# yisol/IDM-VTON

Measured on NVIDIA H100. Metric: try-on images/sec @768x1024, 30 steps, CFG 2.0, higher is better.
Workload: dtype fp16

## Files before the change

idm-vton_b200/csrc/gemm.cu:

```cuda
#include "gemm_common.cuh"
#include "host.h"
#include "wgmma.cuh"

namespace vton {

enum : int { KIND_F16 = 0, KIND_F16IN_F32OUT = 1, KIND_TF32 = 2 };

template <int BN, int STAGES, bool SC>
struct SmemLayout {
  static constexpr int B_BYTES = BN * 128;
  static constexpr int STAGE_BYTES = A_BYTES + B_BYTES;
  static constexpr int LDS = BN + 4;
  static constexpr int STG_BYTES = 128 * LDS * 4;
  static constexpr int RING = STAGES * STAGE_BYTES;
  static constexpr int STG_TOTAL = (SC ? 2 : 1) * STG_BYTES;
  static constexpr int BAR_OFFSET = RING > STG_TOTAL ? RING : STG_TOTAL;
  static constexpr int TOTAL = BAR_OFFSET + 256 + 1024;
};

constexpr int GEMM_THREADS = 288;

template <int BN, int STAGES, bool GEGLU, bool SC, int KIND>
__global__ void __launch_bounds__(GEMM_THREADS, 1)
gemm_conv_kernel(const __grid_constant__ CUtensorMap tmA, const __grid_constant__ CUtensorMap tmB,
                 const __grid_constant__ CUtensorMap tmS0, const __grid_constant__ CUtensorMap tmS1,
                 const __grid_constant__ CUtensorMap tmBs, const GemmParams p) {
  using L = SmemLayout<BN, STAGES, SC>;
  constexpr int KBK = KIND == KIND_TF32 ? 32 : 64;
  extern __shared__ uint8_t smem_raw[];
  const uint32_t smem_base = (smem_u32(smem_raw) + 1023u) & ~1023u;
  float* stg = reinterpret_cast<float*>(smem_raw + (smem_base - smem_u32(smem_raw)));
  const uint32_t bar_base = smem_base + L::BAR_OFFSET;
  auto full_bar = [&](int s) { return bar_base + 8u * s; };
  auto empty_bar = [&](int s) { return bar_base + 8u * (STAGES + s); };

  const int warp = threadIdx.x >> 5;
  const int lane = threadIdx.x & 31;
  const int tile = blockIdx.x;
  const int n_tile = tile % p.n_tiles;
  const int m_tile = tile / p.n_tiles;
  const int n0 = n_tile * BN;
  const int total_slabs = p.slabs_main + (SC ? p.slabs_sc : 0);

  int b0 = 0, y0 = 0, x0 = 0;
  if (p.conv) {
    const int tx = m_tile % p.tiles_x;
    const int ty = (m_tile / p.tiles_x) % p.tiles_y;
    const int tb = m_tile / (p.tiles_x * p.tiles_y);
    x0 = tx * p.bw;
    y0 = ty * p.bh;
    b0 = tb * p.bb;
  }

  if (warp == 8 && lane == 0) {
    tma_prefetch_desc(&tmA);
    tma_prefetch_desc(&tmB);
    if (SC) {
      tma_prefetch_desc(&tmS0);
      tma_prefetch_desc(&tmS1);
      tma_prefetch_desc(&tmBs);
    }
    for (int s = 0; s < STAGES; ++s) {
      mbar_init(full_bar(s), 1);
      mbar_init(empty_bar(s), 2);
    }
    fence_barrier_init();
  }
  pdl_wait();
  __syncthreads();
  pdl_launch_dependents();

  if (warp == 8) {
    if (lane == 0) {
      for (int s = 0; s < total_slabs; ++s) {
        const int stage = s % STAGES;
        const uint32_t phase = (s / STAGES) & 1;
        mbar_wait(empty_bar(stage), phase ^ 1);
        const uint32_t a_dst = smem_base + stage * L::STAGE_BYTES;
        const uint32_t b_dst = a_dst + A_BYTES;
        mbar_expect_tx(full_bar(stage), L::STAGE_BYTES);
        if (s < p.slabs_main) {
          if (p.conv) {
            const int tap = s / p.cin_slabs;
            const int c0 = (s - tap * p.cin_slabs) * KBK;
            const int dy = tap / 3 - 1, dx = tap % 3 - 1;
            tma_load_4d(a_dst, &tmA, full_bar(stage), c0, x0 * p.stride + dx, y0 * p.stride + dy, b0);
            tma_load_2d(b_dst, &tmB, full_bar(stage), c0, tap * p.cout + n0);
          } else {
            tma_load_2d(a_dst, &tmA, full_bar(stage), s * KBK, m_tile * BM);
            tma_load_2d(b_dst, &tmB, full_bar(stage), s * KBK, n0);
          }
        } else {
          const int ss = s - p.slabs_main;
          if (ss < p.sc_split)
            tma_load_4d(a_dst, &tmS0, full_bar(stage), ss * BK, x0, y0, b0);
          else
            tma_load_4d(a_dst, &tmS1, full_bar(stage), (ss - p.sc_split) * BK, x0, y0, b0);
          tma_load_2d(b_dst, &tmBs, full_bar(stage), ss * BK, n0);
        }
      }
    }
    return;
  }

  const int wg = warp >> 2;
  float acc[BN / 2];
  float acc_sc[BN / 2];
  auto run_slabs = [&](float (&accr)[BN / 2], int s_begin, int s_end) {
    for (int s = s_begin; s < s_end; ++s) {
      const int stage = s % STAGES;
      mbar_wait(full_bar(stage), (s / STAGES) & 1);
      const uint32_t a_src = smem_base + stage * L::STAGE_BYTES + wg * (64 * 128);
      const uint32_t b_src = smem_base + stage * L::STAGE_BYTES + A_BYTES;
      wgmma_fence();
#pragma unroll
      for (int k = 0; k < 4; ++k) {
        const uint64_t da = make_gmma_desc_sw128(a_src + k * 32, 0, 1024);
        const uint64_t db = make_gmma_desc_sw128(b_src + k * 32, 0, 1024);
        const int scale_d = (s > s_begin || k > 0) ? 1 : 0;
        if constexpr (KIND == KIND_TF32) {
          WgmmaTF32SS<BN>::mma(accr, da, db, scale_d);
        } else {
          WgmmaF16SS<BN, 0>::mma(accr, da, db, scale_d);
        }
      }
      wgmma_commit();
      wgmma_wait<1>();
      if (s > 0 && (threadIdx.x & 127) == 0) mbar_arrive(empty_bar((s - 1) % STAGES));
    }
  };
  run_slabs(acc, 0, p.slabs_main);
  if constexpr (SC) run_slabs(acc_sc, p.slabs_main, total_slabs);
  wgmma_wait<0>();
  fence_regs(acc);
  if (SC) fence_regs(acc_sc);

  named_bar_sync(1, 256);
  {
    const int r0 = wg * 64 + ((warp & 3) << 4) + (lane >> 2);
    const int cq = (lane & 3) * 2;
#pragma unroll
    for (int i = 0; i < BN / 8; ++i) {
      *reinterpret_cast<float2*>(stg + r0 * L::LDS + i * 8 + cq) = make_float2(acc[4 * i], acc[4 * i + 1]);
      *reinterpret_cast<float2*>(stg + (r0 + 8) * L::LDS + i * 8 + cq) = make_float2(acc[4 * i + 2], acc[4 * i + 3]);
      if (SC) {
        float* s2 = stg + 128 * L::LDS;
        *reinterpret_cast<float2*>(s2 + r0 * L::LDS + i * 8 + cq) = make_float2(acc_sc[4 * i], acc_sc[4 * i + 1]);
        *reinterpret_cast<float2*>(s2 + (r0 + 8) * L::LDS + i * 8 + cq) = make_float2(acc_sc[4 * i + 2], acc_sc[4 * i + 3]);
      }
    }
  }
  named_bar_sync(1, 256);
  const int row = threadIdx.x & 127;
  const int half = threadIdx.x >> 7;
  long long out_row;
  int sample;
  map_row(p, m_tile, row, &out_row, &sample);
  const float* srow = stg + row * L::LDS;
  if (KIND == KIND_F16) {
    epilogue_store<BN, GEGLU>(p, srow, SC ? srow + 128 * L::LDS : nullptr, n_tile, out_row, sample, half, 2);
    return;
  }
  if (out_row < 0) return;
  const float* res_row = p.res_f32 ? p.res_f32 + out_row * p.N : nullptr;
#pragma unroll 1
  for (int c = half; c < BN / 32; c += 2) {
    const int ncol = n0 + c * 32;
    if (ncol >= p.N) continue;
#pragma unroll
    for (int g = 0; g < 8; ++g) {
      float4 v = *reinterpret_cast<const float4*>(srow + c * 32 + g * 4);
      if (p.bias_f32 != nullptr) {
        const float4 b4 = __ldg(reinterpret_cast<const float4*>(p.bias_f32 + ncol + g * 4));
        v.x += b4.x, v.y += b4.y, v.z += b4.z, v.w += b4.w;
      }
      if (res_row != nullptr) {
        const float4 r4 = __ldg(reinterpret_cast<const float4*>(res_row + ncol + g * 4));
        v.x += r4.x, v.y += r4.y, v.z += r4.z, v.w += r4.w;
      }
      *reinterpret_cast<float4*>(p.out_f32 + out_row * p.N + ncol + g * 4) = v;
    }
  }
}

template <int BN, int STAGES, bool GEGLU, bool SC, int KIND>
static int launch_variant(const CUtensorMap& tmA, const CUtensorMap& tmB, const CUtensorMap& tmS0,
                          const CUtensorMap& tmS1, const CUtensorMap& tmBs, const GemmParams& p, int grid,
                          cudaStream_t stream) {
  using L = SmemLayout<BN, STAGES, SC>;
  static_assert(L::TOTAL <= 227 * 1024, "shared memory budget");
  auto kern = gemm_conv_kernel<BN, STAGES, GEGLU, SC, KIND>;
  static bool configured = false;
  if (!configured) {
    VTON_CUDA(cudaFuncSetAttribute(kern, cudaFuncAttributeMaxDynamicSharedMemorySize, L::TOTAL));
    configured = true;
  }
  VTON_CUDA(launch_kernel(kern, dim3(grid), dim3(GEMM_THREADS), L::TOTAL, stream, tmA, tmB, tmS0, tmS1, tmBs, p));
  count_launch();
  return kOk;
}

void set_auto_v2(int) {}
void set_cluster4(int) {}

static int pick_bn(int N, int m_tiles, bool geglu, bool has_shortcut, int force_bn) {
  if (force_bn >= 2000) force_bn -= 2000;
  else if (force_bn >= 1000) force_bn -= 1000;
  auto usable = [&](int bn) {
    if (geglu && ((bn != 256 && bn != 128) || N % bn != 0)) return false;
    if (has_shortcut && bn > 128) return false;
    return true;
  };
  if (force_bn) {
    const bool known = force_bn == 64 || force_bn == 128 || force_bn == 160 || force_bn == 192 || force_bn == 256;
    return known && usable(force_bn) ? force_bn : 0;
  }
  const int sms = num_sms();
  const int cands[5] = {256, 192, 160, 128, 64};
  double best = 1e300;
  int best_bn = 0;
  for (int bn : cands) {
    if (!usable(bn)) continue;
    if (bn != 128 && N % bn != 0 && !(bn == 64 && N < 64)) continue;
    const long long tiles = static_cast<long long>(m_tiles) * cdiv(N, bn);
    const long long waves = (tiles + sms - 1) / sms;
    const double cost = static_cast<double>(waves) * (bn + 64);
    if (cost < best * 0.999) {
      best = cost;
      best_bn = bn;
    }
  }
  return best_bn ? best_bn : 128;
}

static int dispatch(int bn, bool geglu, const CUtensorMap& tmA, const CUtensorMap& tmB, const CUtensorMap& tmS0,
                    const CUtensorMap& tmS1, const CUtensorMap& tmBs, GemmParams& p, int m_tiles,
                    cudaStream_t stream) {
  p.n_tiles = cdiv(p.N, bn);
  const int grid = m_tiles * p.n_tiles;
  if (geglu) {
    if (bn == 128) return launch_variant<128, 6, true, false, KIND_F16>(tmA, tmB, tmS0, tmS1, tmBs, p, grid, stream);
    if (bn == 256) return launch_variant<256, 4, true, false, KIND_F16>(tmA, tmB, tmS0, tmS1, tmBs, p, grid, stream);
    set_last_error("GEGLU epilogue supports BN 128/256 only (got %d)", bn);
    return kErrUnsupported;
  }
  if (p.slabs_sc) {
    if (bn == 64) return launch_variant<64, 8, false, true, KIND_F16>(tmA, tmB, tmS0, tmS1, tmBs, p, grid, stream);
    if (bn == 128) return launch_variant<128, 6, false, true, KIND_F16>(tmA, tmB, tmS0, tmS1, tmBs, p, grid, stream);
    set_last_error("shortcut epilogue supports BN 64/128 only (got %d)", bn);
    return kErrUnsupported;
  }
  switch (bn) {
    case 64: return launch_variant<64, 8, false, false, KIND_F16>(tmA, tmB, tmS0, tmS1, tmBs, p, grid, stream);
    case 128: return launch_variant<128, 6, false, false, KIND_F16>(tmA, tmB, tmS0, tmS1, tmBs, p, grid, stream);
    case 160: return launch_variant<160, 5, false, false, KIND_F16>(tmA, tmB, tmS0, tmS1, tmBs, p, grid, stream);
    case 192: return launch_variant<192, 4, false, false, KIND_F16>(tmA, tmB, tmS0, tmS1, tmBs, p, grid, stream);
    case 256: return launch_variant<256, 4, false, false, KIND_F16>(tmA, tmB, tmS0, tmS1, tmBs, p, grid, stream);
  }
  set_last_error("unsupported BN %d", bn);
  return kErrUnsupported;
}

int gemm_f16_impl(const void* A, long long lda, const void* W, long long ldw, void* out, long long ldo, int M, int N,
                  int K, const void* bias, const void* residual, long long ldr, const void* rowvec, long long ld_rowvec,
                  int rows_per_sample, int flags, int force_bn, cudaStream_t stream) {
  const int geglu = flags & 1;
  VTON_CHECK_ARG(M > 0 && N > 0 && K > 0, "gemm: empty problem M=%d N=%d K=%d", M, N, K);
  VTON_CHECK_ARG(K % 64 == 0, "gemm: K=%d must be a multiple of 64", K);
  VTON_CHECK_ARG(N % 8 == 0 && lda % 8 == 0 && ldw % 8 == 0 && ldo % 8 == 0, "gemm: N/lda/ldw/ldo must be multiples of 8");
  VTON_CHECK_ARG(!geglu || (N % 16 == 0 && !residual && !rowvec), "gemm: bad GEGLU configuration");
  VTON_CHECK_ARG(aligned_to(out, 16) && aligned_to(bias, 16) && aligned_to(residual, 16) && aligned_to(rowvec, 16),
                 "gemm: out/bias/residual/rowvec must be 16-byte aligned");
  VTON_CHECK_ARG((!residual || ldr % 8 == 0) && (!rowvec || ld_rowvec % 8 == 0),
                 "gemm: ldr=%lld / ld_rowvec=%lld must be multiples of 8", ldr, ld_rowvec);
  const int bn = pick_bn(N, cdiv(M, BM), geglu != 0, false, force_bn);
  VTON_CHECK_ARG(bn != 0, "gemm: tile width force_bn=%d unsupported for this problem (N=%d, geglu=%d)", force_bn, N, geglu);
  VTON_CHECK_ARG(!geglu || N % bn == 0, "gemm: GEGLU needs N %% BN == 0 (N=%d, BN=%d)", N, bn);
  CUtensorMap tmA, tmB;
  {
    uint64_t dims[2] = {static_cast<uint64_t>(K), static_cast<uint64_t>(M)};
    uint64_t strides[1] = {static_cast<uint64_t>(lda) * 2};
    uint32_t box[2] = {64, 128};
    if (int e = encode_tmap_f16(&tmA, A, 2, dims, strides, box)) return e;
  }
  {
    uint64_t dims[2] = {static_cast<uint64_t>(K), static_cast<uint64_t>(N)};
    uint64_t strides[1] = {static_cast<uint64_t>(ldw) * 2};
    uint32_t box[2] = {64, static_cast<uint32_t>(bn)};
    if (int e = encode_tmap_f16(&tmB, W, 2, dims, strides, box)) return e;
  }
  GemmParams p{};
  p.out = static_cast<__half*>(out);
  p.ld_out = static_cast<int>(ldo);
  p.M = M;
  p.N = N;
  p.bias = static_cast<const __half*>(bias);
  p.residual = static_cast<const __half*>(residual);
  p.ld_res = static_cast<int>(ldr);
  p.rowvec = static_cast<const __half*>(rowvec);
  p.ld_rowvec = static_cast<int>(ld_rowvec);
  p.rows_per_sample = rows_per_sample;
  p.slabs_main = K / 64;
  p.act_gelu = (flags & 4) ? 2 : ((flags & 2) ? 1 : 0);
  return dispatch(bn, geglu != 0, tmA, tmB, tmA, tmA, tmB, p, cdiv(M, BM), stream);
}

static void pick_box(int B, int H, int W, int* bw, int* bh, int* bb) {
  int w = 1;
  while (w < 128 && W % (w * 2) == 0) w *= 2;
  int h = 1;
  while (w * h < 128 && h * 2 <= H) h *= 2;
  *bw = w;
  *bh = h;
  *bb = 128 / (w * h);
  (void)B;
}

static int encode_nhwc(CUtensorMap* tm, const void* base, int B, int H, int W, int C, int ldc, int bw, int bh, int bb,
                       int pixel_step = 1) {
  uint64_t dims[4] = {static_cast<uint64_t>(C), static_cast<uint64_t>(W), static_cast<uint64_t>(H),
                      static_cast<uint64_t>(B)};
  uint64_t strides[3] = {static_cast<uint64_t>(ldc) * 2, static_cast<uint64_t>(W) * ldc * 2,
                         static_cast<uint64_t>(H) * W * ldc * 2};
  uint32_t box[4] = {64, static_cast<uint32_t>(bw * pixel_step), static_cast<uint32_t>(bh * pixel_step),
                     static_cast<uint32_t>(bb)};
  uint32_t estr[4] = {1, static_cast<uint32_t>(pixel_step), static_cast<uint32_t>(pixel_step), 1};
  return encode_tmap_f16(tm, base, 4, dims, strides, box, pixel_step > 1 ? estr : nullptr);
}

int conv3x3_impl(const void* x, long long ldx, int B, int Hin, int Win, int Cin, const void* w, int Cout, const void* bias,
                 const void* temb, long long ld_temb, const void* sc0, int C0, const void* sc1, int C1, const void* w_sc,
                 const void* bias_sc, const void* residual, long long ldr, void* out, long long ldo, int force_bn,
                 int stride, cudaStream_t stream) {
  VTON_CHECK_ARG(B > 0 && Hin > 0 && Win > 0, "conv3x3: empty input");
  VTON_CHECK_ARG(stride == 1 || stride == 2, "conv3x3: stride %d unsupported", stride);
  VTON_CHECK_ARG(stride == 1 || (!w_sc && !residual), "conv3x3: stride 2 has no shortcut / residual form");
  const int H = (Hin - 1) / stride + 1, W = (Win - 1) / stride + 1;
  VTON_CHECK_ARG(Cin % 64 == 0, "conv3x3: Cin=%d must be a multiple of 64 (pad channels)", Cin);
  VTON_CHECK_ARG(Cout % 8 == 0 && ldo % 8 == 0 && ldx % 8 == 0, "conv3x3: Cout/ldo/ldx must be multiples of 8");
  VTON_CHECK_ARG(C0 % 64 == 0 && C1 % 64 == 0, "conv3x3: shortcut source channels must be multiples of 64");
  VTON_CHECK_ARG(!(w_sc && residual), "conv3x3: shortcut conv and identity residual are exclusive");
  VTON_CHECK_ARG(aligned_to(out, 16) && aligned_to(bias, 16) && aligned_to(temb, 16) && aligned_to(bias_sc, 16) &&
                     aligned_to(residual, 16),
                 "conv3x3: out/bias/temb/bias_sc/residual must be 16-byte aligned");
  VTON_CHECK_ARG((!residual || ldr % 8 == 0) && (!temb || ld_temb % 8 == 0),
                 "conv3x3: ldr=%lld / ld_temb=%lld must be multiples of 8", ldr, ld_temb);
  int bw, bh, bb;
  pick_box(B, H, W, &bw, &bh, &bb);
  const int m_tiles_est = (W / bw) * cdiv(H, bh) * cdiv(B, bb);
  const int bn = pick_bn(Cout, m_tiles_est, false, w_sc != nullptr, force_bn);
  VTON_CHECK_ARG(bn != 0, "conv3x3: tile width force_bn=%d unsupported (a fused shortcut takes 64 or 128)", force_bn);
  CUtensorMap tmA, tmB, tmS0, tmS1, tmBs;
  VTON_CHECK_ARG(stride == 1 || (bw * 2 <= 256 && bh * 2 <= 256), "conv3x3: stride-2 box too large");
  if (int e = encode_nhwc(&tmA, x, B, Hin, Win, Cin, static_cast<int>(ldx), bw, bh, bb, stride)) return e;
  {
    uint64_t dims[2] = {static_cast<uint64_t>(Cin), static_cast<uint64_t>(9) * Cout};
    uint64_t strides[1] = {static_cast<uint64_t>(Cin) * 2};
    uint32_t box[2] = {64, static_cast<uint32_t>(bn)};
    if (int e = encode_tmap_f16(&tmB, w, 2, dims, strides, box)) return e;
  }
  tmS0 = tmA;
  tmS1 = tmA;
  tmBs = tmB;
  GemmParams p{};
  if (w_sc) {
    VTON_CHECK_ARG(sc0 && C0 > 0, "conv3x3: shortcut needs a source");
    if (int e = encode_nhwc(&tmS0, sc0, B, H, W, C0, C0, bw, bh, bb)) return e;
    if (sc1 && C1 > 0) {
      if (int e = encode_nhwc(&tmS1, sc1, B, H, W, C1, C1, bw, bh, bb)) return e;
    }
    const int Csc = C0 + (sc1 ? C1 : 0);
    uint64_t dims[2] = {static_cast<uint64_t>(Csc), static_cast<uint64_t>(Cout)};
    uint64_t strides[1] = {static_cast<uint64_t>(Csc) * 2};
    uint32_t box[2] = {64, static_cast<uint32_t>(bn)};
    if (int e = encode_tmap_f16(&tmBs, w_sc, 2, dims, strides, box)) return e;
    p.slabs_sc = Csc / 64;
    p.sc_split = C0 / 64;
  }
  p.out = static_cast<__half*>(out);
  p.ld_out = static_cast<int>(ldo);
  p.M = B * H * W;
  p.N = Cout;
  p.bias = static_cast<const __half*>(bias);
  p.bias_sc = static_cast<const __half*>(bias_sc);
  p.residual = static_cast<const __half*>(residual);
  p.ld_res = static_cast<int>(ldr);
  p.rowvec = static_cast<const __half*>(temb);
  p.ld_rowvec = static_cast<int>(ld_temb);
  p.slabs_main = 9 * (Cin / 64);
  p.conv = 1;
  p.stride = stride;
  p.H = H;
  p.W = W;
  p.B = B;
  p.bw = bw;
  p.bh = bh;
  p.bb = bb;
  p.tiles_x = W / bw;
  p.tiles_y = cdiv(H, bh);
  p.cin_slabs = Cin / 64;
  p.cout = Cout;
  const int m_tiles = p.tiles_x * p.tiles_y * cdiv(B, bb);
  return dispatch(bn, false, tmA, tmB, tmS0, tmS1, tmBs, p, m_tiles, stream);
}

int conv3x3_f32_impl(const void* x, int B, int H, int W, int Cin, const void* w, int Cout, const void* bias,
                     const void* residual, void* out, int in_fp16, cudaStream_t stream) {
  VTON_CHECK_ARG(B > 0 && H > 0 && W > 0, "conv3x3_f32: empty input");
  VTON_CHECK_ARG(Cin % 32 == 0 && Cout % 32 == 0 && Cout >= 64, "conv3x3_f32: Cin=%d / Cout=%d must be multiples of 32 (Cout >= 64)", Cin, Cout);
  VTON_CHECK_ARG(!in_fp16 || Cin % 64 == 0, "conv3x3_f32: fp16 operands need Cin=%d to be a multiple of 64", Cin);
  VTON_CHECK_ARG(x && w && out, "conv3x3_f32: null pointer");
  const int esz = in_fp16 ? 2 : 4;
  const int bk = in_fp16 ? 64 : 32;
  int bw, bh, bb;
  pick_box(B, H, W, &bw, &bh, &bb);
  VTON_CHECK_ARG(bw * bh * bb == 128 && bw >= 8, "conv3x3_f32: W=%d H=%d cannot be tiled into 128-pixel boxes", W, H);
  const int m_tiles = (W / bw) * cdiv(H, bh) * cdiv(B, bb);
  const int bn = pick_bn(Cout, m_tiles, false, false, Cout % 256 == 0 ? 256 : 128);
  CUtensorMap tmA, tmB;
  {
    uint64_t dims[4] = {static_cast<uint64_t>(Cin), static_cast<uint64_t>(W), static_cast<uint64_t>(H), static_cast<uint64_t>(B)};
    uint64_t strides[3] = {static_cast<uint64_t>(Cin) * esz, static_cast<uint64_t>(W) * Cin * esz,
                           static_cast<uint64_t>(H) * W * Cin * esz};
    uint32_t box[4] = {static_cast<uint32_t>(bk), static_cast<uint32_t>(bw), static_cast<uint32_t>(bh), static_cast<uint32_t>(bb)};
    if (int e = in_fp16 ? encode_tmap_f16(&tmA, x, 4, dims, strides, box) : encode_tmap_f32(&tmA, x, 4, dims, strides, box)) return e;
  }
  {
    uint64_t dims[2] = {static_cast<uint64_t>(Cin), static_cast<uint64_t>(9) * Cout};
    uint64_t strides[1] = {static_cast<uint64_t>(Cin) * esz};
    uint32_t box[2] = {static_cast<uint32_t>(bk), static_cast<uint32_t>(bn)};
    if (int e = in_fp16 ? encode_tmap_f16(&tmB, w, 2, dims, strides, box) : encode_tmap_f32(&tmB, w, 2, dims, strides, box)) return e;
  }
  GemmParams p{};
  p.out_f32 = static_cast<float*>(out);
  p.bias_f32 = static_cast<const float*>(bias);
  p.res_f32 = static_cast<const float*>(residual);
  p.M = B * H * W;
  p.N = Cout;
  p.slabs_main = 9 * (Cin / bk);
  p.conv = 1;
  p.stride = 1;
  p.H = H;
  p.W = W;
  p.B = B;
  p.bw = bw;
  p.bh = bh;
  p.bb = bb;
  p.tiles_x = W / bw;
  p.tiles_y = cdiv(H, bh);
  p.cin_slabs = Cin / bk;
  p.cout = Cout;
  p.n_tiles = cdiv(Cout, bn);
  const int grid = m_tiles * p.n_tiles;
  if (in_fp16) {
    if (bn == 256) return launch_variant<256, 4, false, false, KIND_F16IN_F32OUT>(tmA, tmB, tmA, tmA, tmB, p, grid, stream);
    return launch_variant<128, 6, false, false, KIND_F16IN_F32OUT>(tmA, tmB, tmA, tmA, tmB, p, grid, stream);
  }
  if (bn == 256) return launch_variant<256, 4, false, false, KIND_TF32>(tmA, tmB, tmA, tmA, tmB, p, grid, stream);
  return launch_variant<128, 6, false, false, KIND_TF32>(tmA, tmB, tmA, tmA, tmB, p, grid, stream);
}

}
```

idm-vton_b200/csrc/gemm_common.cuh:

```cuda
#pragma once
#include "common.cuh"

namespace vton {

struct GemmParams {
  __half* out;
  int ld_out;
  int M, N;
  const __half* bias;
  const __half* bias_sc;
  const __half* residual;
  int ld_res;
  const __half* rowvec;
  int ld_rowvec;
  int rows_per_sample;
  int slabs_main;
  int slabs_sc;
  int sc_split;
  int conv;
  int H, W, B;
  int bw, bh, bb;
  int tiles_x, tiles_y;
  int cin_slabs;
  int cout;
  int n_tiles;
  int act_gelu;
  int stride;
  float* out_f32;
  const float* bias_f32;
  const float* res_f32;
};

constexpr int BM = 128;
constexpr int BK = 64;
constexpr int A_BYTES = BM * BK * 2;

__device__ __forceinline__ void map_row(const GemmParams& p, int m_tile, int r_local, long long* out_row, int* sample) {
  *out_row = -1;
  if (p.conv) {
    const int tx = m_tile % p.tiles_x;
    const int ty = (m_tile / p.tiles_x) % p.tiles_y;
    const int tb = m_tile / (p.tiles_x * p.tiles_y);
    const int lx = r_local % p.bw;
    const int ly = (r_local / p.bw) % p.bh;
    const int lb = r_local / (p.bw * p.bh);
    const int b = tb * p.bb + lb, y = ty * p.bh + ly, x = tx * p.bw + lx;
    if (b < p.B && y < p.H && x < p.W) *out_row = (static_cast<long long>(b) * p.H + y) * p.W + x;
    *sample = b;
  } else {
    const int m = m_tile * BM + r_local;
    if (m < p.M) *out_row = m;
    *sample = p.rows_per_sample > 0 ? m / p.rows_per_sample : 0;
  }
}

enum : int { EPI_BIAS = 1, EPI_ROWVEC = 2, EPI_RES = 4, EPI_RUNTIME = 8 };

__device__ __forceinline__ float gelu_erf_fast(float x) {
  const float ax = fabsf(x) * 0.70710678118654752f;
  const float t = __fdividef(1.0f, fmaf(0.3275911f, ax, 1.0f));
  float poly = fmaf(t, 1.061405429f, -1.453152027f);
  poly = fmaf(poly, t, 1.421413741f);
  poly = fmaf(poly, t, -0.284496736f);
  poly = fmaf(poly, t, 0.254829592f);
  poly *= t;
  float e;
  const float arg = -ax * ax * 1.4426950408889634f;
  asm("ex2.approx.ftz.f32 %0, %1;" : "=f"(e) : "f"(arg));
  const float erf_abs = fmaf(-poly, e, 1.0f);
  const float erf_v = copysignf(erf_abs, x);
  return 0.5f * x * (1.0f + erf_v);
}

template <int BN, bool GEGLU, int EPI>
__device__ __forceinline__ void epilogue_load(const GemmParams& p, const float* row, const float* row_sc, int c,
                                              uint32_t (&acc)[32], uint32_t (&acc2)[32]) {
#pragma unroll
  for (int i = 0; i < 32; i += 4) {
    const float4 v = *reinterpret_cast<const float4*>(row + c * 32 + i);
    acc[i] = __float_as_uint(v.x), acc[i + 1] = __float_as_uint(v.y), acc[i + 2] = __float_as_uint(v.z), acc[i + 3] = __float_as_uint(v.w);
  }
  const float* src2 = GEGLU ? row + BN / 2 : (((EPI & EPI_RUNTIME) && p.slabs_sc) ? row_sc : nullptr);
  if (src2 != nullptr) {
#pragma unroll
    for (int i = 0; i < 32; i += 4) {
      const float4 v = *reinterpret_cast<const float4*>(src2 + c * 32 + i);
      acc2[i] = __float_as_uint(v.x), acc2[i + 1] = __float_as_uint(v.y), acc2[i + 2] = __float_as_uint(v.z), acc2[i + 3] = __float_as_uint(v.w);
    }
  }
}

__device__ __forceinline__ void add_h8(float (&v)[8], const __half* src) {
  const uint4 u = *reinterpret_cast<const uint4*>(src);
  const uint32_t w[4] = {u.x, u.y, u.z, u.w};
#pragma unroll
  for (int j = 0; j < 4; ++j) {
    const float2 a = unpack_h2(w[j]);
    v[2 * j] += a.x;
    v[2 * j + 1] += a.y;
  }
}
__device__ __forceinline__ void add_u4(float (&v)[8], const uint4 u) {
  const uint32_t w[4] = {u.x, u.y, u.z, u.w};
#pragma unroll
  for (int j = 0; j < 4; ++j) {
    const float2 a = unpack_h2(w[j]);
    v[2 * j] += a.x;
    v[2 * j + 1] += a.y;
  }
}
__device__ __forceinline__ void round_add_u4(float (&v)[8], const uint4 u) {
  const uint32_t w[4] = {u.x, u.y, u.z, u.w};
#pragma unroll
  for (int j = 0; j < 4; ++j) {
    const float2 a = unpack_h2(w[j]);
    v[2 * j] = round_h(v[2 * j]) + a.x;
    v[2 * j + 1] = round_h(v[2 * j + 1]) + a.y;
  }
}
__device__ __forceinline__ void round_add_h8(float (&v)[8], const __half* src) {
  const uint4 u = *reinterpret_cast<const uint4*>(src);
  const uint32_t w[4] = {u.x, u.y, u.z, u.w};
#pragma unroll
  for (int j = 0; j < 4; ++j) {
    const float2 a = unpack_h2(w[j]);
    v[2 * j] = round_h(v[2 * j]) + a.x;
    v[2 * j + 1] = round_h(v[2 * j + 1]) + a.y;
  }
}

template <int BN, bool GEGLU, int EPI>
__device__ __forceinline__ void epilogue_math(const GemmParams& p, int n_tile, long long out_row, int sample, int c,
                                              const uint32_t (&acc)[32], const uint32_t (&acc2)[32], uint32_t (&pk)[16],
                                              const uint4* res_pre = nullptr, const uint4* bias_pre = nullptr) {
  constexpr bool RT = (EPI & EPI_RUNTIME) != 0;
  const bool has_bias = RT ? (p.bias != nullptr) : ((EPI & EPI_BIAS) != 0);
  const bool has_rowvec = RT ? (p.rowvec != nullptr) : ((EPI & EPI_ROWVEC) != 0);
  const bool has_res = RT ? (p.residual != nullptr) : ((EPI & EPI_RES) != 0);
  const int n0 = n_tile * BN;
  const int out_n0 = GEGLU ? n_tile * (BN / 2) : n0;
  const int out_N = GEGLU ? p.N / 2 : p.N;
  const __half* rowvec_row = (has_rowvec && out_row >= 0) ? p.rowvec + static_cast<long long>(sample) * p.ld_rowvec : nullptr;
  const __half* res_row = (has_res && out_row >= 0) ? p.residual + out_row * p.ld_res : nullptr;
#pragma unroll
  for (int g = 0; g < 4; ++g) {
    const int ncol = out_n0 + c * 32 + g * 8;
    const bool col_ok = ncol < out_N;
    float v[8];
#pragma unroll
    for (int j = 0; j < 8; ++j) v[j] = __uint_as_float(acc[g * 8 + j]);
    if (GEGLU) {
      const int bcol = n0 + c * 32 + g * 8;
      float gt[8];
#pragma unroll
      for (int j = 0; j < 8; ++j) gt[j] = __uint_as_float(acc2[g * 8 + j]);
      if (p.bias && col_ok) {
        add_h8(v, p.bias + bcol);
        add_h8(gt, p.bias + bcol + BN / 2);
      }
#pragma unroll
      for (int j = 0; j < 8; ++j) {
        const float hv = round_h(v[j]);
        const float gv = round_h(gt[j]);
        v[j] = hv * round_h(gelu_erf_fast(gv));
      }
    } else {
      if (bias_pre != nullptr) {
        if (has_bias) add_u4(v, bias_pre[g]);
      } else if (has_bias && col_ok) {
        add_h8(v, p.bias + ncol);
      }
      if (RT && p.act_gelu) {
#pragma unroll 1
        for (int j = 0; j < 8; ++j) {
          const float x = round_h(v[j]);
          v[j] = p.act_gelu == 2 ? __fdividef(x, 1.0f + __expf(-1.702f * x)) : gelu_erf_fast(x);
        }
      }
      if (has_rowvec && col_ok && rowvec_row != nullptr) round_add_h8(v, rowvec_row + ncol);
      if (RT && p.slabs_sc) {
        float s[8];
#pragma unroll
        for (int j = 0; j < 8; ++j) s[j] = __uint_as_float(acc2[g * 8 + j]);
        if (p.bias_sc && col_ok) add_h8(s, p.bias_sc + ncol);
#pragma unroll
        for (int j = 0; j < 8; ++j) v[j] = round_h(s[j]) + round_h(v[j]);
      }
      if (res_pre != nullptr) {
        if (has_res) round_add_u4(v, res_pre[g]);
      } else if (has_res && col_ok && res_row != nullptr) {
        round_add_h8(v, res_row + ncol);
      }
    }
    pk[g * 4 + 0] = pack_h2(v[0], v[1]);
    pk[g * 4 + 1] = pack_h2(v[2], v[3]);
    pk[g * 4 + 2] = pack_h2(v[4], v[5]);
    pk[g * 4 + 3] = pack_h2(v[6], v[7]);
  }
}

template <int BN, bool GEGLU>
__device__ __forceinline__ void epilogue_store(const GemmParams& p, const float* row, const float* row_sc, int n_tile,
                                               long long out_row, int sample, int c_first, int c_step) {
  constexpr int OUT_COLS = GEGLU ? BN / 2 : BN;
  const int out_n0 = GEGLU ? n_tile * (BN / 2) : n_tile * BN;
  const int out_N = GEGLU ? p.N / 2 : p.N;
#pragma unroll 1
  for (int c = c_first; c < OUT_COLS / 32; c += c_step) {
    if (out_row < 0 || out_n0 + c * 32 >= out_N) continue;
    uint32_t acc[32], acc2[32];
    uint32_t pk[16];
    epilogue_load<BN, GEGLU, EPI_RUNTIME>(p, row, row_sc, c, acc, acc2);
    epilogue_math<BN, GEGLU, EPI_RUNTIME>(p, n_tile, out_row, sample, c, acc, acc2, pk);
#pragma unroll
    for (int g = 0; g < 4; ++g) {
      const int ncol = out_n0 + c * 32 + g * 8;
      if (ncol >= out_N) continue;
      *reinterpret_cast<uint4*>(p.out + out_row * p.ld_out + ncol) =
          make_uint4(pk[g * 4], pk[g * 4 + 1], pk[g * 4 + 2], pk[g * 4 + 3]);
    }
  }
}

__device__ __forceinline__ void tma_store_2d(const CUtensorMap* m, uint32_t src, int c0, int c1) {
  asm volatile("cp.async.bulk.tensor.2d.global.shared::cta.bulk_group [%0, {%2, %3}], [%1];"
               ::"l"(reinterpret_cast<uint64_t>(m)), "r"(src), "r"(c0), "r"(c1)
               : "memory");
}
__device__ __forceinline__ void tma_store_4d(const CUtensorMap* m, uint32_t src, int c0, int c1, int c2, int c3) {
  asm volatile("cp.async.bulk.tensor.4d.global.shared::cta.bulk_group [%0, {%2, %3, %4, %5}], [%1];"
               ::"l"(reinterpret_cast<uint64_t>(m)), "r"(src), "r"(c0), "r"(c1), "r"(c2), "r"(c3)
               : "memory");
}
__device__ __forceinline__ void tma_store_commit() { asm volatile("cp.async.bulk.commit_group;" ::: "memory"); }
template <int N>
__device__ __forceinline__ void tma_store_wait_read() {
  asm volatile("cp.async.bulk.wait_group.read %0;" ::"n"(N) : "memory");
}
template <int N>
__device__ __forceinline__ void tma_store_wait_all() {
  asm volatile("cp.async.bulk.wait_group %0;" ::"n"(N) : "memory");
}

}
```

Before: 0.8103.

## Make GEMM persistent with register-direct epilogue and TMA output stores

Turns the GEMM/conv kernel into a persistent kernel that loops over tiles with a global stage counter, so the producer warp can prefetch the next tile while the consumers finish the current one. The epilogue now computes bias, activation, rowvec, shortcut and residual straight from the wgmma accumulators. Results go into swizzled fp16 staging chunks in shared memory that TMA stores write out, replacing the full fp32 shared-memory staging pass. The PDL trigger moves to the last tile, and the tile-size cost model penalizes BN=256 for non-GEGLU shapes. The staging area is sized to whatever shared memory the ring leaves free, which adds more barrier round-trips and makes the epilogue index math more complex.

```diff
diff --git a/idm-vton_b200/csrc/gemm.cu b/idm-vton_b200/csrc/gemm.cu
--- a/idm-vton_b200/csrc/gemm.cu
+++ b/idm-vton_b200/csrc/gemm.cu
@@ -6,16 +6,23 @@
 
 enum : int { KIND_F16 = 0, KIND_F16IN_F32OUT = 1, KIND_TF32 = 2 };
 
-template <int BN, int STAGES, bool SC>
+constexpr int SMEM_LIMIT = 227 * 1024;
+constexpr int SMEM_EXTRA = 256 + 1024;
+
+template <int BN, int STAGES, bool GEGLU, int KIND>
 struct SmemLayout {
   static constexpr int B_BYTES = BN * 128;
   static constexpr int STAGE_BYTES = A_BYTES + B_BYTES;
-  static constexpr int LDS = BN + 4;
-  static constexpr int STG_BYTES = 128 * LDS * 4;
   static constexpr int RING = STAGES * STAGE_BYTES;
-  static constexpr int STG_TOTAL = (SC ? 2 : 1) * STG_BYTES;
-  static constexpr int BAR_OFFSET = RING > STG_TOTAL ? RING : STG_TOTAL;
-  static constexpr int TOTAL = BAR_OFFSET + 256 + 1024;
+  static constexpr int OUT_COLS = GEGLU ? BN / 2 : BN;
+  static constexpr int CHUNKS = KIND == KIND_F16 ? OUT_COLS / 32 : 0;
+  static constexpr int CHUNK_BYTES = 128 * 64;
+  static constexpr int FIT = (SMEM_LIMIT - SMEM_EXTRA - RING) / CHUNK_BYTES;
+  static constexpr int STG_CHUNKS = CHUNKS < FIT ? CHUNKS : FIT;
+  static constexpr int BAR_OFFSET = RING + STG_CHUNKS * CHUNK_BYTES;
+  static constexpr int TOTAL = BAR_OFFSET + SMEM_EXTRA;
+  static_assert(KIND != KIND_F16 || STG_CHUNKS >= 1, "no room for the output staging tile");
+  static_assert(TOTAL <= SMEM_LIMIT, "shared memory budget");
 };
 
 constexpr int GEMM_THREADS = 288;
@@ -24,33 +31,29 @@
 __global__ void __launch_bounds__(GEMM_THREADS, 1)
 gemm_conv_kernel(const __grid_constant__ CUtensorMap tmA, const __grid_constant__ CUtensorMap tmB,
                  const __grid_constant__ CUtensorMap tmS0, const __grid_constant__ CUtensorMap tmS1,
-                 const __grid_constant__ CUtensorMap tmBs, const GemmParams p) {
-  using L = SmemLayout<BN, STAGES, SC>;
+                 const __grid_constant__ CUtensorMap tmBs, const __grid_constant__ CUtensorMap tmO,
+                 const GemmParams p) {
+  using L = SmemLayout<BN, STAGES, GEGLU, KIND>;
   constexpr int KBK = KIND == KIND_TF32 ? 32 : 64;
   extern __shared__ uint8_t smem_raw[];
   const uint32_t smem_base = (smem_u32(smem_raw) + 1023u) & ~1023u;
-  float* stg = reinterpret_cast<float*>(smem_raw + (smem_base - smem_u32(smem_raw)));
+  const uint32_t stg_base = smem_base + L::RING;
   const uint32_t bar_base = smem_base + L::BAR_OFFSET;
   auto full_bar = [&](int s) { return bar_base + 8u * s; };
   auto empty_bar = [&](int s) { return bar_base + 8u * (STAGES + s); };
 
   const int warp = threadIdx.x >> 5;
   const int lane = threadIdx.x & 31;
-  const int tile = blockIdx.x;
-  const int n_tile = tile % p.n_tiles;
-  const int m_tile = tile / p.n_tiles;
-  const int n0 = n_tile * BN;
+  const int tiles = p.m_tiles * p.n_tiles;
   const int total_slabs = p.slabs_main + (SC ? p.slabs_sc : 0);
-
-  int b0 = 0, y0 = 0, x0 = 0;
-  if (p.conv) {
+  auto conv_origin = [&](int m_tile, int* b0, int* y0, int* x0) {
     const int tx = m_tile % p.tiles_x;
     const int ty = (m_tile / p.tiles_x) % p.tiles_y;
     const int tb = m_tile / (p.tiles_x * p.tiles_y);
-    x0 = tx * p.bw;
-    y0 = ty * p.bh;
-    b0 = tb * p.bb;
-  }
+    *x0 = tx * p.bw;
+    *y0 = ty * p.bh;
+    *b0 = tb * p.bb;
+  };
 
   if (warp == 8 && lane == 0) {
     tma_prefetch_desc(&tmA);
@@ -60,6 +63,7 @@
       tma_prefetch_desc(&tmS1);
       tma_prefetch_desc(&tmBs);
     }
+    if (KIND == KIND_F16) tma_prefetch_desc(&tmO);
     for (int s = 0; s < STAGES; ++s) {
       mbar_init(full_bar(s), 1);
       mbar_init(empty_bar(s), 2);
@@ -68,35 +72,41 @@
   }
   pdl_wait();
   __syncthreads();
-  pdl_launch_dependents();
 
   if (warp == 8) {
     if (lane == 0) {
-      for (int s = 0; s < total_slabs; ++s) {
-        const int stage = s % STAGES;
-        const uint32_t phase = (s / STAGES) & 1;
-        mbar_wait(empty_bar(stage), phase ^ 1);
-        const uint32_t a_dst = smem_base + stage * L::STAGE_BYTES;
-        const uint32_t b_dst = a_dst + A_BYTES;
-        mbar_expect_tx(full_bar(stage), L::STAGE_BYTES);
-        if (s < p.slabs_main) {
-          if (p.conv) {
-            const int tap = s / p.cin_slabs;
-            const int c0 = (s - tap * p.cin_slabs) * KBK;
-            const int dy = tap / 3 - 1, dx = tap % 3 - 1;
-            tma_load_4d(a_dst, &tmA, full_bar(stage), c0, x0 * p.stride + dx, y0 * p.stride + dy, b0);
-            tma_load_2d(b_dst, &tmB, full_bar(stage), c0, tap * p.cout + n0);
+      uint32_t g = 0;
+      for (int tile = blockIdx.x; tile < tiles; tile += gridDim.x) {
+        int m_tile, n_tile, b0 = 0, y0 = 0, x0 = 0;
+        tile_coords(p, tile, &m_tile, &n_tile);
+        if (p.conv) conv_origin(m_tile, &b0, &y0, &x0);
+        const int n0 = n_tile * BN;
+        for (int s = 0; s < total_slabs; ++s, ++g) {
+          const int stage = g % STAGES;
+          const uint32_t phase = (g / STAGES) & 1;
+          mbar_wait(empty_bar(stage), phase ^ 1);
+          const uint32_t a_dst = smem_base + stage * L::STAGE_BYTES;
+          const uint32_t b_dst = a_dst + A_BYTES;
+          mbar_expect_tx(full_bar(stage), L::STAGE_BYTES);
+          if (s < p.slabs_main) {
+            if (p.conv) {
+              const int tap = s / p.cin_slabs;
+              const int c0 = (s - tap * p.cin_slabs) * KBK;
+              const int dy = tap / 3 - 1, dx = tap % 3 - 1;
+              tma_load_4d(a_dst, &tmA, full_bar(stage), c0, x0 * p.stride + dx, y0 * p.stride + dy, b0);
+              tma_load_2d(b_dst, &tmB, full_bar(stage), c0, tap * p.cout + n0);
+            } else {
+              tma_load_2d(a_dst, &tmA, full_bar(stage), s * KBK, m_tile * BM);
+              tma_load_2d(b_dst, &tmB, full_bar(stage), s * KBK, n0);
+            }
           } else {
-            tma_load_2d(a_dst, &tmA, full_bar(stage), s * KBK, m_tile * BM);
-            tma_load_2d(b_dst, &tmB, full_bar(stage), s * KBK, n0);
+            const int ss = s - p.slabs_main;
+            if (ss < p.sc_split)
+              tma_load_4d(a_dst, &tmS0, full_bar(stage), ss * BK, x0, y0, b0);
+            else
+              tma_load_4d(a_dst, &tmS1, full_bar(stage), (ss - p.sc_split) * BK, x0, y0, b0);
+            tma_load_2d(b_dst, &tmBs, full_bar(stage), ss * BK, n0);
           }
-        } else {
-          const int ss = s - p.slabs_main;
-          if (ss < p.sc_split)
-            tma_load_4d(a_dst, &tmS0, full_bar(stage), ss * BK, x0, y0, b0);
-          else
-            tma_load_4d(a_dst, &tmS1, full_bar(stage), (ss - p.sc_split) * BK, x0, y0, b0);
-          tma_load_2d(b_dst, &tmBs, full_bar(stage), ss * BK, n0);
         }
       }
     }
@@ -104,12 +114,17 @@
   }
 
   const int wg = warp >> 2;
+  const int r0 = wg * 64 + ((warp & 3) << 4) + (lane >> 2);
+  const int cq = (lane & 3) * 2;
+  const bool store_thread = threadIdx.x == 0;
   float acc[BN / 2];
   float acc_sc[BN / 2];
+  uint32_t g0 = 0;
   auto run_slabs = [&](float (&accr)[BN / 2], int s_begin, int s_end) {
     for (int s = s_begin; s < s_end; ++s) {
-      const int stage = s % STAGES;
-      mbar_wait(full_bar(stage), (s / STAGES) & 1);
+      const uint32_t g = g0 + s;
+      const int stage = g % STAGES;
+      mbar_wait(full_bar(stage), (g / STAGES) & 1);
       const uint32_t a_src = smem_base + stage * L::STAGE_BYTES + wg * (64 * 128);
       const uint32_t b_src = smem_base + stage * L::STAGE_BYTES + A_BYTES;
       wgmma_fence();
@@ -126,76 +141,107 @@
       }
       wgmma_commit();
       wgmma_wait<1>();
-      if (s > 0 && (threadIdx.x & 127) == 0) mbar_arrive(empty_bar((s - 1) % STAGES));
+      if (s > 0 && (threadIdx.x & 127) == 0) mbar_arrive(empty_bar((g - 1) % STAGES));
     }
   };
-  run_slabs(acc, 0, p.slabs_main);
-  if constexpr (SC) run_slabs(acc_sc, p.slabs_main, total_slabs);
-  wgmma_wait<0>();
-  fence_regs(acc);
-  if (SC) fence_regs(acc_sc);
-
-  named_bar_sync(1, 256);
-  {
-    const int r0 = wg * 64 + ((warp & 3) << 4) + (lane >> 2);
-    const int cq = (lane & 3) * 2;
+
+  for (int tile = blockIdx.x; tile < tiles; tile += gridDim.x) {
+    int m_tile, n_tile, b0 = 0, y0 = 0, x0 = 0;
+    tile_coords(p, tile, &m_tile, &n_tile);
+    if (!GEGLU && p.conv) conv_origin(m_tile, &b0, &y0, &x0);
+    const int n0 = n_tile * BN;
+
+    run_slabs(acc, 0, p.slabs_main);
+    if constexpr (SC) run_slabs(acc_sc, p.slabs_main, total_slabs);
+    wgmma_wait<0>();
+    fence_regs(acc);
+    if (SC) fence_regs(acc_sc);
+    if ((threadIdx.x & 127) == 0) mbar_arrive(empty_bar((g0 + total_slabs - 1) % STAGES));
+    g0 += total_slabs;
+    if (tile + static_cast<int>(gridDim.x) >= tiles) pdl_launch_dependents();
+
+    int out_row[2];
+    int sample[2];
+    map_row(p, m_tile, r0, &out_row[0], &sample[0]);
+    map_row(p, m_tile, r0 + 8, &out_row[1], &sample[1]);
+
+    if constexpr (KIND != KIND_F16) {
 #pragma unroll
-    for (int i = 0; i < BN / 8; ++i) {
-      *reinterpret_cast<float2*>(stg + r0 * L::LDS + i * 8 + cq) = make_float2(acc[4 * i], acc[4 * i + 1]);
-      *reinterpret_cast<float2*>(stg + (r0 + 8) * L::LDS + i * 8 + cq) = make_float2(acc[4 * i + 2], acc[4 * i + 3]);
-      if (SC) {
-        float* s2 = stg + 128 * L::LDS;
-        *reinterpret_cast<float2*>(s2 + r0 * L::LDS + i * 8 + cq) = make_float2(acc_sc[4 * i], acc_sc[4 * i + 1]);
-        *reinterpret_cast<float2*>(s2 + (r0 + 8) * L::LDS + i * 8 + cq) = make_float2(acc_sc[4 * i + 2], acc_sc[4 * i + 3]);
+      for (int i = 0; i < BN / 8; ++i) {
+        const int col = n0 + i * 8 + cq;
+        if (col >= p.N) continue;
+        float2 b = make_float2(0.f, 0.f);
+        if (p.bias_f32 != nullptr) b = __ldg(reinterpret_cast<const float2*>(p.bias_f32 + col));
+#pragma unroll
+        for (int h = 0; h < 2; ++h) {
+          if (out_row[h] < 0) continue;
+          float2 v = make_float2(acc[4 * i + 2 * h], acc[4 * i + 2 * h + 1]);
+          if (p.bias_f32 != nullptr) v.x += b.x, v.y += b.y;
+          if (p.res_f32 != nullptr) {
+            const float2 r = __ldg(reinterpret_cast<const float2*>(p.res_f32 + static_cast<long long>(out_row[h]) * p.N + col));
+            v.x += r.x, v.y += r.y;
+          }
+          *reinterpret_cast<float2*>(p.out_f32 + static_cast<long long>(out_row[h]) * p.N + col) = v;
+        }
       }
-    }
-  }
-  named_bar_sync(1, 256);
-  const int row = threadIdx.x & 127;
-  const int half = threadIdx.x >> 7;
-  long long out_row;
-  int sample;
-  map_row(p, m_tile, row, &out_row, &sample);
-  const float* srow = stg + row * L::LDS;
-  if (KIND == KIND_F16) {
-    epilogue_store<BN, GEGLU>(p, srow, SC ? srow + 128 * L::LDS : nullptr, n_tile, out_row, sample, half, 2);
-    return;
-  }
-  if (out_row < 0) return;
-  const float* res_row = p.res_f32 ? p.res_f32 + out_row * p.N : nullptr;
-#pragma unroll 1
-  for (int c = half; c < BN / 32; c += 2) {
-    const int ncol = n0 + c * 32;
-    if (ncol >= p.N) continue;
+    } else {
+      const int out_n0 = GEGLU ? n_tile * (BN / 2) : n0;
 #pragma unroll
-    for (int g = 0; g < 8; ++g) {
-      float4 v = *reinterpret_cast<const float4*>(srow + c * 32 + g * 4);
-      if (p.bias_f32 != nullptr) {
-        const float4 b4 = __ldg(reinterpret_cast<const float4*>(p.bias_f32 + ncol + g * 4));
-        v.x += b4.x, v.y += b4.y, v.z += b4.z, v.w += b4.w;
+      for (int c_begin = 0; c_begin < L::CHUNKS; c_begin += L::STG_CHUNKS) {
+        constexpr int c_step = L::STG_CHUNKS;
+        if (store_thread) tma_store_wait_read<0>();
+        named_bar_sync(1, 256);
+#pragma unroll
+        for (int i = c_begin * 4; i < (c_begin + c_step < L::CHUNKS ? c_begin + c_step : L::CHUNKS) * 4; ++i) {
+          const uint32_t chunk = stg_base + ((i / 4) - c_begin) * L::CHUNK_BYTES;
+#pragma unroll
+          for (int h = 0; h < 2; ++h) {
+            const int r = r0 + 8 * h;
+            uint32_t packed;
+            if constexpr (GEGLU) {
+              const int j = 4 * (i + BN / 16) + 2 * h;
+              packed = epilogue_pair_geglu<BN>(p, acc[4 * i + 2 * h], acc[4 * i + 2 * h + 1], acc[j], acc[j + 1],
+                                               n0 + i * 8 + cq);
+            } else {
+              packed = epilogue_pair<SC>(p, acc[4 * i + 2 * h], acc[4 * i + 2 * h + 1], SC ? acc_sc[4 * i + 2 * h] : 0.f,
+                                         SC ? acc_sc[4 * i + 2 * h + 1] : 0.f, n0 + i * 8 + cq, out_row[h], sample[h]);
+            }
+            const uint32_t addr = chunk + r * 64 + ((((i & 3) ^ (r >> 1)) & 3) << 4) + cq * 2;
+            asm volatile("st.shared.u32 [%0], %1;" ::"r"(addr), "r"(packed) : "memory");
+          }
+        }
+        fence_proxy_async_smem();
+        named_bar_sync(1, 256);
+        if (store_thread) {
+          for (int c = c_begin; c < c_begin + c_step && c < L::CHUNKS; ++c) {
+            const uint32_t src = stg_base + (c - c_begin) * L::CHUNK_BYTES;
+            if (!GEGLU && p.conv)
+              tma_store_4d(&tmO, src, out_n0 + c * 32, x0, y0, b0);
+            else
+              tma_store_2d(&tmO, src, out_n0 + c * 32, m_tile * BM);
+          }
+          tma_store_commit();
+        }
       }
-      if (res_row != nullptr) {
-        const float4 r4 = __ldg(reinterpret_cast<const float4*>(res_row + ncol + g * 4));
-        v.x += r4.x, v.y += r4.y, v.z += r4.z, v.w += r4.w;
-      }
-      *reinterpret_cast<float4*>(p.out_f32 + out_row * p.N + ncol + g * 4) = v;
-    }
-  }
+    }
+  }
+  if (KIND == KIND_F16 && store_thread) tma_store_wait_all<0>();
 }
 
 template <int BN, int STAGES, bool GEGLU, bool SC, int KIND>
 static int launch_variant(const CUtensorMap& tmA, const CUtensorMap& tmB, const CUtensorMap& tmS0,
-                          const CUtensorMap& tmS1, const CUtensorMap& tmBs, const GemmParams& p, int grid,
+                          const CUtensorMap& tmS1, const CUtensorMap& tmBs, const CUtensorMap& tmO, const GemmParams& p,
                           cudaStream_t stream) {
-  using L = SmemLayout<BN, STAGES, SC>;
-  static_assert(L::TOTAL <= 227 * 1024, "shared memory budget");
+  using L = SmemLayout<BN, STAGES, GEGLU, KIND>;
+  const int tiles = p.m_tiles * p.n_tiles;
+  const int grid = tiles < num_sms() ? tiles : num_sms();
   auto kern = gemm_conv_kernel<BN, STAGES, GEGLU, SC, KIND>;
   static bool configured = false;
   if (!configured) {
     VTON_CUDA(cudaFuncSetAttribute(kern, cudaFuncAttributeMaxDynamicSharedMemorySize, L::TOTAL));
     configured = true;
   }
-  VTON_CUDA(launch_kernel(kern, dim3(grid), dim3(GEMM_THREADS), L::TOTAL, stream, tmA, tmB, tmS0, tmS1, tmBs, p));
+  VTON_CUDA(launch_kernel(kern, dim3(grid), dim3(GEMM_THREADS), L::TOTAL, stream, tmA, tmB, tmS0, tmS1, tmBs, tmO, p));
   count_launch();
   return kOk;
 }
@@ -224,7 +270,7 @@
     if (bn != 128 && N % bn != 0 && !(bn == 64 && N < 64)) continue;
     const long long tiles = static_cast<long long>(m_tiles) * cdiv(N, bn);
     const long long waves = (tiles + sms - 1) / sms;
-    const double cost = static_cast<double>(waves) * (bn + 64);
+    const double cost = static_cast<double>(waves) * (bn + 64) * (bn == 256 && !geglu ? 1.15 : 1.0);
     if (cost < best * 0.999) {
       best = cost;
       best_bn = bn;
@@ -234,28 +280,28 @@
 }
 
 static int dispatch(int bn, bool geglu, const CUtensorMap& tmA, const CUtensorMap& tmB, const CUtensorMap& tmS0,
-                    const CUtensorMap& tmS1, const CUtensorMap& tmBs, GemmParams& p, int m_tiles,
-                    cudaStream_t stream) {
+                    const CUtensorMap& tmS1, const CUtensorMap& tmBs, const CUtensorMap& tmO, GemmParams& p,
+                    int m_tiles, cudaStream_t stream) {
   p.n_tiles = cdiv(p.N, bn);
-  const int grid = m_tiles * p.n_tiles;
+  p.m_tiles = m_tiles;
   if (geglu) {
-    if (bn == 128) return launch_variant<128, 6, true, false, KIND_F16>(tmA, tmB, tmS0, tmS1, tmBs, p, grid, stream);
-    if (bn == 256) return launch_variant<256, 4, true, false, KIND_F16>(tmA, tmB, tmS0, tmS1, tmBs, p, grid, stream);
+    if (bn == 128) return launch_variant<128, 6, true, false, KIND_F16>(tmA, tmB, tmS0, tmS1, tmBs, tmO, p, stream);
+    if (bn == 256) return launch_variant<256, 4, true, false, KIND_F16>(tmA, tmB, tmS0, tmS1, tmBs, tmO, p, stream);
     set_last_error("GEGLU epilogue supports BN 128/256 only (got %d)", bn);
     return kErrUnsupported;
   }
   if (p.slabs_sc) {
-    if (bn == 64) return launch_variant<64, 8, false, true, KIND_F16>(tmA, tmB, tmS0, tmS1, tmBs, p, grid, stream);
-    if (bn == 128) return launch_variant<128, 6, false, true, KIND_F16>(tmA, tmB, tmS0, tmS1, tmBs, p, grid, stream);
+    if (bn == 64) return launch_variant<64, 8, false, true, KIND_F16>(tmA, tmB, tmS0, tmS1, tmBs, tmO, p, stream);
+    if (bn == 128) return launch_variant<128, 6, false, true, KIND_F16>(tmA, tmB, tmS0, tmS1, tmBs, tmO, p, stream);
     set_last_error("shortcut epilogue supports BN 64/128 only (got %d)", bn);
     return kErrUnsupported;
   }
   switch (bn) {
-    case 64: return launch_variant<64, 8, false, false, KIND_F16>(tmA, tmB, tmS0, tmS1, tmBs, p, grid, stream);
-    case 128: return launch_variant<128, 6, false, false, KIND_F16>(tmA, tmB, tmS0, tmS1, tmBs, p, grid, stream);
-    case 160: return launch_variant<160, 5, false, false, KIND_F16>(tmA, tmB, tmS0, tmS1, tmBs, p, grid, stream);
-    case 192: return launch_variant<192, 4, false, false, KIND_F16>(tmA, tmB, tmS0, tmS1, tmBs, p, grid, stream);
-    case 256: return launch_variant<256, 4, false, false, KIND_F16>(tmA, tmB, tmS0, tmS1, tmBs, p, grid, stream);
+    case 64: return launch_variant<64, 8, false, false, KIND_F16>(tmA, tmB, tmS0, tmS1, tmBs, tmO, p, stream);
+    case 128: return launch_variant<128, 6, false, false, KIND_F16>(tmA, tmB, tmS0, tmS1, tmBs, tmO, p, stream);
+    case 160: return launch_variant<160, 5, false, false, KIND_F16>(tmA, tmB, tmS0, tmS1, tmBs, tmO, p, stream);
+    case 192: return launch_variant<192, 4, false, false, KIND_F16>(tmA, tmB, tmS0, tmS1, tmBs, tmO, p, stream);
+    case 256: return launch_variant<256, 4, false, false, KIND_F16>(tmA, tmB, tmS0, tmS1, tmBs, tmO, p, stream);
   }
   set_last_error("unsupported BN %d", bn);
   return kErrUnsupported;
@@ -289,6 +335,13 @@
     uint32_t box[2] = {64, static_cast<uint32_t>(bn)};
     if (int e = encode_tmap_f16(&tmB, W, 2, dims, strides, box)) return e;
   }
+  CUtensorMap tmO;
+  {
+    uint64_t dims[2] = {static_cast<uint64_t>(geglu ? N / 2 : N), static_cast<uint64_t>(M)};
+    uint64_t strides[1] = {static_cast<uint64_t>(ldo) * 2};
+    uint32_t box[2] = {32, 128};
+    if (int e = encode_tmap_f16(&tmO, out, 2, dims, strides, box, nullptr, 64)) return e;
+  }
   GemmParams p{};
   p.out = static_cast<__half*>(out);
   p.ld_out = static_cast<int>(ldo);
@@ -302,7 +355,7 @@
   p.rows_per_sample = rows_per_sample;
   p.slabs_main = K / 64;
   p.act_gelu = (flags & 4) ? 2 : ((flags & 2) ? 1 : 0);
-  return dispatch(bn, geglu != 0, tmA, tmB, tmA, tmA, tmB, p, cdiv(M, BM), stream);
+  return dispatch(bn, geglu != 0, tmA, tmB, tmA, tmA, tmB, tmO, p, cdiv(M, BM), stream);
 }
 
 static void pick_box(int B, int H, int W, int* bw, int* bh, int* bb) {
@@ -350,8 +403,16 @@
   const int m_tiles_est = (W / bw) * cdiv(H, bh) * cdiv(B, bb);
   const int bn = pick_bn(Cout, m_tiles_est, false, w_sc != nullptr, force_bn);
   VTON_CHECK_ARG(bn != 0, "conv3x3: tile width force_bn=%d unsupported (a fused shortcut takes 64 or 128)", force_bn);
-  CUtensorMap tmA, tmB, tmS0, tmS1, tmBs;
+  CUtensorMap tmA, tmB, tmS0, tmS1, tmBs, tmO;
   VTON_CHECK_ARG(stride == 1 || (bw * 2 <= 256 && bh * 2 <= 256), "conv3x3: stride-2 box too large");
+  {
+    uint64_t dims[4] = {static_cast<uint64_t>(Cout), static_cast<uint64_t>(W), static_cast<uint64_t>(H),
+                        static_cast<uint64_t>(B)};
+    uint64_t strides[3] = {static_cast<uint64_t>(ldo) * 2, static_cast<uint64_t>(W) * ldo * 2,
+                           static_cast<uint64_t>(H) * W * ldo * 2};
+    uint32_t box[4] = {32, static_cast<uint32_t>(bw), static_cast<uint32_t>(bh), static_cast<uint32_t>(bb)};
+    if (int e = encode_tmap_f16(&tmO, out, 4, dims, strides, box, nullptr, 64)) return e;
+  }
   if (int e = encode_nhwc(&tmA, x, B, Hin, Win, Cin, static_cast<int>(ldx), bw, bh, bb, stride)) return e;
   {
     uint64_t dims[2] = {static_cast<uint64_t>(Cin), static_cast<uint64_t>(9) * Cout};
@@ -401,7 +462,7 @@
   p.cin_slabs = Cin / 64;
   p.cout = Cout;
   const int m_tiles = p.tiles_x * p.tiles_y * cdiv(B, bb);
-  return dispatch(bn, false, tmA, tmB, tmS0, tmS1, tmBs, p, m_tiles, stream);
+  return dispatch(bn, false, tmA, tmB, tmS0, tmS1, tmBs, tmO, p, m_tiles, stream);
 }
 
 int conv3x3_f32_impl(const void* x, int B, int H, int W, int Cin, const void* w, int Cout, const void* bias,
@@ -451,13 +512,13 @@
   p.cin_slabs = Cin / bk;
   p.cout = Cout;
   p.n_tiles = cdiv(Cout, bn);
-  const int grid = m_tiles * p.n_tiles;
+  p.m_tiles = m_tiles;
   if (in_fp16) {
-    if (bn == 256) return launch_variant<256, 4, false, false, KIND_F16IN_F32OUT>(tmA, tmB, tmA, tmA, tmB, p, grid, stream);
-    return launch_variant<128, 6, false, false, KIND_F16IN_F32OUT>(tmA, tmB, tmA, tmA, tmB, p, grid, stream);
-  }
-  if (bn == 256) return launch_variant<256, 4, false, false, KIND_TF32>(tmA, tmB, tmA, tmA, tmB, p, grid, stream);
-  return launch_variant<128, 6, false, false, KIND_TF32>(tmA, tmB, tmA, tmA, tmB, p, grid, stream);
-}
-
-}
+    if (bn == 256) return launch_variant<256, 4, false, false, KIND_F16IN_F32OUT>(tmA, tmB, tmA, tmA, tmB, tmA, p, stream);
+    return launch_variant<128, 6, false, false, KIND_F16IN_F32OUT>(tmA, tmB, tmA, tmA, tmB, tmA, p, stream);
+  }
+  if (bn == 256) return launch_variant<256, 4, false, false, KIND_TF32>(tmA, tmB, tmA, tmA, tmB, tmA, p, stream);
+  return launch_variant<128, 6, false, false, KIND_TF32>(tmA, tmB, tmA, tmA, tmB, tmA, p, stream);
+}
+
+}
diff --git a/idm-vton_b200/csrc/gemm_common.cuh b/idm-vton_b200/csrc/gemm_common.cuh
--- a/idm-vton_b200/csrc/gemm_common.cuh
+++ b/idm-vton_b200/csrc/gemm_common.cuh
@@ -24,6 +24,7 @@
   int cin_slabs;
   int cout;
   int n_tiles;
+  int m_tiles;
   int act_gelu;
   int stride;
   float* out_f32;
@@ -35,7 +36,18 @@
 constexpr int BK = 64;
 constexpr int A_BYTES = BM * BK * 2;
 
-__device__ __forceinline__ void map_row(const GemmParams& p, int m_tile, int r_local, long long* out_row, int* sample) {
+constexpr int GROUP_M = 8;
+__device__ __forceinline__ void tile_coords(const GemmParams& p, int tile, int* m_tile, int* n_tile) {
+  const int per_group = GROUP_M * p.n_tiles;
+  const int group = tile / per_group;
+  const int first_m = group * GROUP_M;
+  const int rows = min(GROUP_M, p.m_tiles - first_m);
+  const int t = tile - group * per_group;
+  *m_tile = first_m + t % rows;
+  *n_tile = t / rows;
+}
+
+__device__ __forceinline__ void map_row(const GemmParams& p, int m_tile, int r_local, int* out_row, int* sample) {
   *out_row = -1;
   if (p.conv) {
     const int tx = m_tile % p.tiles_x;
@@ -45,7 +57,7 @@
     const int ly = (r_local / p.bw) % p.bh;
     const int lb = r_local / (p.bw * p.bh);
     const int b = tb * p.bb + lb, y = ty * p.bh + ly, x = tx * p.bw + lx;
-    if (b < p.B && y < p.H && x < p.W) *out_row = (static_cast<long long>(b) * p.H + y) * p.W + x;
+    if (b < p.B && y < p.H && x < p.W) *out_row = (b * p.H + y) * p.W + x;
     *sample = b;
   } else {
     const int m = m_tile * BM + r_local;
@@ -53,8 +65,6 @@
     *sample = p.rows_per_sample > 0 ? m / p.rows_per_sample : 0;
   }
 }
-
-enum : int { EPI_BIAS = 1, EPI_ROWVEC = 2, EPI_RES = 4, EPI_RUNTIME = 8 };
 
 __device__ __forceinline__ float gelu_erf_fast(float x) {
   const float ax = fabsf(x) * 0.70710678118654752f;
@@ -72,154 +82,61 @@
   return 0.5f * x * (1.0f + erf_v);
 }
 
-template <int BN, bool GEGLU, int EPI>
-__device__ __forceinline__ void epilogue_load(const GemmParams& p, const float* row, const float* row_sc, int c,
-                                              uint32_t (&acc)[32], uint32_t (&acc2)[32]) {
-#pragma unroll
-  for (int i = 0; i < 32; i += 4) {
-    const float4 v = *reinterpret_cast<const float4*>(row + c * 32 + i);
-    acc[i] = __float_as_uint(v.x), acc[i + 1] = __float_as_uint(v.y), acc[i + 2] = __float_as_uint(v.z), acc[i + 3] = __float_as_uint(v.w);
-  }
-  const float* src2 = GEGLU ? row + BN / 2 : (((EPI & EPI_RUNTIME) && p.slabs_sc) ? row_sc : nullptr);
-  if (src2 != nullptr) {
-#pragma unroll
-    for (int i = 0; i < 32; i += 4) {
-      const float4 v = *reinterpret_cast<const float4*>(src2 + c * 32 + i);
-      acc2[i] = __float_as_uint(v.x), acc2[i + 1] = __float_as_uint(v.y), acc2[i + 2] = __float_as_uint(v.z), acc2[i + 3] = __float_as_uint(v.w);
-    }
-  }
+__device__ __forceinline__ float2 ldg_h2(const __half* src) {
+  return unpack_h2(__ldg(reinterpret_cast<const unsigned int*>(src)));
 }
 
-__device__ __forceinline__ void add_h8(float (&v)[8], const __half* src) {
-  const uint4 u = *reinterpret_cast<const uint4*>(src);
-  const uint32_t w[4] = {u.x, u.y, u.z, u.w};
-#pragma unroll
-  for (int j = 0; j < 4; ++j) {
-    const float2 a = unpack_h2(w[j]);
-    v[2 * j] += a.x;
-    v[2 * j + 1] += a.y;
+template <bool SC>
+__device__ __forceinline__ uint32_t epilogue_pair(const GemmParams& p, float v0, float v1, float s0, float s1, int col,
+                                                  int out_row, int sample) {
+  const bool col_ok = col < p.N;
+  const bool row_ok = col_ok && out_row >= 0;
+  if (p.bias && col_ok) {
+    const float2 b = ldg_h2(p.bias + col);
+    v0 += b.x;
+    v1 += b.y;
   }
-}
-__device__ __forceinline__ void add_u4(float (&v)[8], const uint4 u) {
-  const uint32_t w[4] = {u.x, u.y, u.z, u.w};
-#pragma unroll
-  for (int j = 0; j < 4; ++j) {
-    const float2 a = unpack_h2(w[j]);
-    v[2 * j] += a.x;
-    v[2 * j + 1] += a.y;
+  if (p.act_gelu) {
+    const float x0 = round_h(v0), x1 = round_h(v1);
+    v0 = p.act_gelu == 2 ? __fdividef(x0, 1.0f + __expf(-1.702f * x0)) : gelu_erf_fast(x0);
+    v1 = p.act_gelu == 2 ? __fdividef(x1, 1.0f + __expf(-1.702f * x1)) : gelu_erf_fast(x1);
   }
-}
-__device__ __forceinline__ void round_add_u4(float (&v)[8], const uint4 u) {
-  const uint32_t w[4] = {u.x, u.y, u.z, u.w};
-#pragma unroll
-  for (int j = 0; j < 4; ++j) {
-    const float2 a = unpack_h2(w[j]);
-    v[2 * j] = round_h(v[2 * j]) + a.x;
-    v[2 * j + 1] = round_h(v[2 * j + 1]) + a.y;
+  if (p.rowvec && row_ok) {
+    const float2 t = ldg_h2(p.rowvec + static_cast<long long>(sample) * p.ld_rowvec + col);
+    v0 = round_h(v0) + t.x;
+    v1 = round_h(v1) + t.y;
   }
-}
-__device__ __forceinline__ void round_add_h8(float (&v)[8], const __half* src) {
-  const uint4 u = *reinterpret_cast<const uint4*>(src);
-  const uint32_t w[4] = {u.x, u.y, u.z, u.w};
-#pragma unroll
-  for (int j = 0; j < 4; ++j) {
-    const float2 a = unpack_h2(w[j]);
-    v[2 * j] = round_h(v[2 * j]) + a.x;
-    v[2 * j + 1] = round_h(v[2 * j + 1]) + a.y;
+  if (SC) {
+    if (p.bias_sc && col_ok) {
+      const float2 b = ldg_h2(p.bias_sc + col);
+      s0 += b.x;
+      s1 += b.y;
+    }
+    v0 = round_h(s0) + round_h(v0);
+    v1 = round_h(s1) + round_h(v1);
   }
+  if (p.residual && row_ok) {
+    const float2 r = ldg_h2(p.residual + static_cast<long long>(out_row) * p.ld_res + col);
+    v0 = round_h(v0) + r.x;
+    v1 = round_h(v1) + r.y;
+  }
+  return pack_h2(v0, v1);
 }
 
-template <int BN, bool GEGLU, int EPI>
-__device__ __forceinline__ void epilogue_math(const GemmParams& p, int n_tile, long long out_row, int sample, int c,
-                                              const uint32_t (&acc)[32], const uint32_t (&acc2)[32], uint32_t (&pk)[16],
-                                              const uint4* res_pre = nullptr, const uint4* bias_pre = nullptr) {
-  constexpr bool RT = (EPI & EPI_RUNTIME) != 0;
-  const bool has_bias = RT ? (p.bias != nullptr) : ((EPI & EPI_BIAS) != 0);
-  const bool has_rowvec = RT ? (p.rowvec != nullptr) : ((EPI & EPI_ROWVEC) != 0);
-  const bool has_res = RT ? (p.residual != nullptr) : ((EPI & EPI_RES) != 0);
-  const int n0 = n_tile * BN;
-  const int out_n0 = GEGLU ? n_tile * (BN / 2) : n0;
-  const int out_N = GEGLU ? p.N / 2 : p.N;
-  const __half* rowvec_row = (has_rowvec && out_row >= 0) ? p.rowvec + static_cast<long long>(sample) * p.ld_rowvec : nullptr;
-  const __half* res_row = (has_res && out_row >= 0) ? p.residual + out_row * p.ld_res : nullptr;
-#pragma unroll
-  for (int g = 0; g < 4; ++g) {
-    const int ncol = out_n0 + c * 32 + g * 8;
-    const bool col_ok = ncol < out_N;
-    float v[8];
-#pragma unroll
-    for (int j = 0; j < 8; ++j) v[j] = __uint_as_float(acc[g * 8 + j]);
-    if (GEGLU) {
-      const int bcol = n0 + c * 32 + g * 8;
-      float gt[8];
-#pragma unroll
-      for (int j = 0; j < 8; ++j) gt[j] = __uint_as_float(acc2[g * 8 + j]);
-      if (p.bias && col_ok) {
-        add_h8(v, p.bias + bcol);
-        add_h8(gt, p.bias + bcol + BN / 2);
-      }
-#pragma unroll
-      for (int j = 0; j < 8; ++j) {
-        const float hv = round_h(v[j]);
-        const float gv = round_h(gt[j]);
-        v[j] = hv * round_h(gelu_erf_fast(gv));
-      }
-    } else {
-      if (bias_pre != nullptr) {
-        if (has_bias) add_u4(v, bias_pre[g]);
-      } else if (has_bias && col_ok) {
-        add_h8(v, p.bias + ncol);
-      }
-      if (RT && p.act_gelu) {
-#pragma unroll 1
-        for (int j = 0; j < 8; ++j) {
-          const float x = round_h(v[j]);
-          v[j] = p.act_gelu == 2 ? __fdividef(x, 1.0f + __expf(-1.702f * x)) : gelu_erf_fast(x);
-        }
-      }
-      if (has_rowvec && col_ok && rowvec_row != nullptr) round_add_h8(v, rowvec_row + ncol);
-      if (RT && p.slabs_sc) {
-        float s[8];
-#pragma unroll
-        for (int j = 0; j < 8; ++j) s[j] = __uint_as_float(acc2[g * 8 + j]);
-        if (p.bias_sc && col_ok) add_h8(s, p.bias_sc + ncol);
-#pragma unroll
-        for (int j = 0; j < 8; ++j) v[j] = round_h(s[j]) + round_h(v[j]);
-      }
-      if (res_pre != nullptr) {
-        if (has_res) round_add_u4(v, res_pre[g]);
-      } else if (has_res && col_ok && res_row != nullptr) {
-        round_add_h8(v, res_row + ncol);
-      }
-    }
-    pk[g * 4 + 0] = pack_h2(v[0], v[1]);
-    pk[g * 4 + 1] = pack_h2(v[2], v[3]);
-    pk[g * 4 + 2] = pack_h2(v[4], v[5]);
-    pk[g * 4 + 3] = pack_h2(v[6], v[7]);
+template <int BN>
+__device__ __forceinline__ uint32_t epilogue_pair_geglu(const GemmParams& p, float v0, float v1, float g0, float g1,
+                                                        int bcol) {
+  if (p.bias) {
+    const float2 b = ldg_h2(p.bias + bcol);
+    const float2 bg = ldg_h2(p.bias + bcol + BN / 2);
+    v0 += b.x;
+    v1 += b.y;
+    g0 += bg.x;
+    g1 += bg.y;
   }
-}
-
-template <int BN, bool GEGLU>
-__device__ __forceinline__ void epilogue_store(const GemmParams& p, const float* row, const float* row_sc, int n_tile,
-                                               long long out_row, int sample, int c_first, int c_step) {
-  constexpr int OUT_COLS = GEGLU ? BN / 2 : BN;
-  const int out_n0 = GEGLU ? n_tile * (BN / 2) : n_tile * BN;
-  const int out_N = GEGLU ? p.N / 2 : p.N;
-#pragma unroll 1
-  for (int c = c_first; c < OUT_COLS / 32; c += c_step) {
-    if (out_row < 0 || out_n0 + c * 32 >= out_N) continue;
-    uint32_t acc[32], acc2[32];
-    uint32_t pk[16];
-    epilogue_load<BN, GEGLU, EPI_RUNTIME>(p, row, row_sc, c, acc, acc2);
-    epilogue_math<BN, GEGLU, EPI_RUNTIME>(p, n_tile, out_row, sample, c, acc, acc2, pk);
-#pragma unroll
-    for (int g = 0; g < 4; ++g) {
-      const int ncol = out_n0 + c * 32 + g * 8;
-      if (ncol >= out_N) continue;
-      *reinterpret_cast<uint4*>(p.out + out_row * p.ld_out + ncol) =
-          make_uint4(pk[g * 4], pk[g * 4 + 1], pk[g * 4 + 2], pk[g * 4 + 3]);
-    }
-  }
+  v0 = round_h(v0) * round_h(gelu_erf_fast(round_h(g0)));
+  v1 = round_h(v1) * round_h(gelu_erf_fast(round_h(g1)));
+  return pack_h2(v0, v1);
 }
 
 __device__ __forceinline__ void tma_store_2d(const CUtensorMap* m, uint32_t src, int c0, int c1) {
```

Result: no change. 0.8104 (median of 6 runs) (+0.0%).
